# applied-ai-lab/genesis

Hardware: AMD Instinct MI355X
Metric: training images/sec (fwd+bwd+GECO step), GENESIS-V2 K=7 64x64 (higher is better)
Workload: dtype f32

## Files before the change

### genesis_amd/csrc/gx_kq.hip

```cpp
#include "gx_common.h"

#include <cstdlib>

#ifndef GX_KQ_ABL
#define GX_KQ_ABL 0
#endif
#ifndef GX_KQ_VAR
#define GX_KQ_VAR 0
#endif
#ifndef GX_QH_ABL
#define GX_QH_ABL 0
#endif

namespace {

enum { Q_C3 = 0, Q_DT0 = 1, Q_DT1 = 2, Q_DG = 3, Q_DT0H = 4, Q_DT1H = 5, Q_DGH = 6, Q_C3H = 7, Q_C5H = 8 };

template <int MODE> struct QCfg;
template <> struct QCfg<Q_C3> {
    static constexpr int NPH = 1, NT = 9, MAXT = 9, NCLS = 1;
    static constexpr bool PLANE_PER_PHASE = false;
    __host__ __device__ static constexpr int ntaps(int) { return 9; }
    __host__ __device__ static constexpr int tbase(int) { return 0; }
    __host__ __device__ static constexpr int ro(int, int i) { return i / 3; }
    __host__ __device__ static constexpr int co(int, int i) { return i % 3; }
    __host__ __device__ static constexpr int cls(int, int) { return 0; }
};
template <> struct QCfg<Q_DT0> {
    static constexpr int NPH = 3, NT = 15, MAXT = 5, NCLS = 2;
    static constexpr bool PLANE_PER_PHASE = false;
    __host__ __device__ static constexpr int ntaps(int) { return 5; }
    __host__ __device__ static constexpr int tbase(int p) { return 5 * p; }
    __host__ __device__ static constexpr int ro(int p, int) { return 2 - p; }
    __host__ __device__ static constexpr int co(int, int i) { return 2 - i / 2; }
    __host__ __device__ static constexpr int cls(int, int i) { return i & 1; }
};
template <> struct QCfg<Q_DT1> {
    static constexpr int NPH = 2, NT = 10, MAXT = 5, NCLS = 2;
    static constexpr bool PLANE_PER_PHASE = false;
    __host__ __device__ static constexpr int ntaps(int) { return 5; }
    __host__ __device__ static constexpr int tbase(int p) { return 5 * p; }
    __host__ __device__ static constexpr int ro(int p, int) { return 2 - p; }
    __host__ __device__ static constexpr int co(int, int i) { return 2 - i / 2; }
    __host__ __device__ static constexpr int cls(int, int i) { return i & 1; }
};
template <> struct QCfg<Q_DG> {
    static constexpr int NPH = 4, NT = 25, MAXT = 9, NCLS = 1;
    static constexpr bool PLANE_PER_PHASE = true;
    __host__ __device__ static constexpr int nkw(int p) { return 3 - (p & 1); }
    __host__ __device__ static constexpr int ntaps(int p) { return (3 - (p >> 1)) * (3 - (p & 1)); }
    __host__ __device__ static constexpr int tbase(int p) { return p == 0 ? 0 : (p == 1 ? 9 : (p == 2 ? 15 : 21)); }
    __host__ __device__ static constexpr int ro(int p, int i) { return i / nkw(p); }
    __host__ __device__ static constexpr int co(int p, int i) { return i % nkw(p); }
    __host__ __device__ static constexpr int cls(int, int) { return 0; }
};

template <int PA> struct QCfgDTH {
    static constexpr int NKH = PA ? 2 : 3;
    static constexpr int NPH = 2 * NKH, NT = 5 * NKH, MAXT = 3, NCLS = 2;
    static constexpr bool PLANE_PER_PHASE = false;
    __host__ __device__ static constexpr int ntaps(int ph) { return (ph & 1) ? 2 : 3; }
    __host__ __device__ static constexpr int tbase(int ph) { return 5 * (ph >> 1) + 3 * (ph & 1); }
    __host__ __device__ static constexpr int ro(int ph, int) { return 2 - (ph >> 1); }
    __host__ __device__ static constexpr int co(int ph, int j) { return 2 - (3 * (ph & 1) + j) / 2; }
// ... 136 lines not shown
    {                                                                                                  \
        const int toff_ = C::ro(PH, i_) * HS4 + C::co(PH, i_) * 4;                                     \
        _Pragma("unroll") for (int mi_ = 0; mi_ < MI; ++mi_)                                           \
            fa[set_][mi_] = *reinterpret_cast<const f32x4*>(wb + (i_) * 512 + a_lane + mi_ * 128);     \
        fb[set_][0] = *reinterpret_cast<const f32x4*>(ib + b_lane0 + toff_);                           \
        fb[set_][1] = *reinterpret_cast<const f32x4*>(ib + b_lane1 + toff_);                           \
    }
    GX_Q_READ(0, 0)
    __builtin_amdgcn_sched_group_barrier(0x100, 2 + MI, 0);
#pragma unroll
    for (int i = 0; i < nt; ++i) {
        const int cur = i & 1;
        if (i + 1 < nt) GX_Q_READ(i + 1, cur ^ 1)
        const int cl = C::cls(PH, i);
#pragma unroll
        for (int j = 0; j < 4; ++j) {
#pragma unroll
            for (int mi = 0; mi < MI; ++mi) {
                acc[cl][mi][0] = __builtin_amdgcn_mfma_f32_32x32x2f32(fa[cur][mi][j], fb[cur][0][j], acc[cl][mi][0], 0, 0, 0);
                acc[cl][mi][1] = __builtin_amdgcn_mfma_f32_32x32x2f32(fa[cur][mi][j], fb[cur][1][j], acc[cl][mi][1], 0, 0, 0);
            }
        }
#if GX_KQ_VAR == 1
        for (int r = 0; r < 4; ++r) {
            __builtin_amdgcn_sched_group_barrier(0x008, 4, 0);
            if (i + 1 < nt) __builtin_amdgcn_sched_group_barrier(0x100, 1, 0);
        }
#elif GX_KQ_VAR == 2
#else
        if (i + 1 < nt) __builtin_amdgcn_sched_group_barrier(0x100, 2 + MI, 0);
        __builtin_amdgcn_sched_group_barrier(0x008, 8 * MI, 0);
#endif
    }
#undef GX_Q_READ
}

__device__ __forceinline__ float q_amax_parts(const float* __restrict__ parts, int n) {
    float m = 0.f;
    int i0 = 0;
    if ((reinterpret_cast<uintptr_t>(parts) & 15) == 0) {
        const int n4 = n >> 2;
        for (int i = threadIdx.x & 63; i < n4; i += 64) {
            const f32x4 v = reinterpret_cast<const f32x4*>(parts)[i];
            m = fmaxf(fmaxf(m, fmaxf(v[0], v[1])), fmaxf(v[2], v[3]));
        }
        i0 = n4 << 2;
    }
    for (int i = i0 + (threadIdx.x & 63); i < n; i += 64) m = fmaxf(m, parts[i]);
#pragma unroll
    for (int o = 32; o > 0; o >>= 1) m = fmaxf(m, __shfl_xor(m, o, 64));
    return __builtin_bit_cast(float, __builtin_amdgcn_readfirstlane(__builtin_bit_cast(int, m)));
}

template <int MODE, int NQ, bool STATS, int MI = 2, int PF = PF_B6, bool TAP = false>
__device__ __forceinline__ void q_body(const float* __restrict__ in, const float* __restrict__ wp,
                                       const float* __restrict__ bias, float* __restrict__ out, const QGeom& g,
                                       float* lds, const int bx, const int by, const int par_a, const int mh = 0) {
    using C = QCfg<MODE>;
    constexpr bool F16 = PF == PF_F3, B1 = PF == PF_B1;
    constexpr bool B16 = MODE >= Q_DT0H;
    constexpr int NPH = C::NPH, NT = C::NT, MAXT = C::MAXT, NCLS = C::NCLS;
    constexpr int NW = (MAXT * 128 + 255) / 256;
    constexpr int WSLOT = NW * 1024;
    constexpr int ISLOT = NQ * 1024;

    const int tid = threadIdx.x, lane = tid & 63, wave = tid >> 6;
    const bool RT = MODE == Q_C3H && g.rt_tw > 0;
    const int TH = RT ? g.rt_th : 1 << g.lTH, TW = RT ? g.rt_tw : 1 << g.lTW, G = RT ? 1 : 1 << g.lG;
    constexpr int HL = MODE == Q_C5H ? 2 : 1;
    const int HS = TW + 2 * HL;
    const int CHS = G * (TH + 2 * HL) * HS;
    float* const ibuf0 = lds;
    float* const wbuf0 = lds + 2 * ISLOT;

    int tile = bx;
    const int tw_i = tile % g.tiles_w; tile /= g.tiles_w;
    const int th_i = tile % g.tiles_h; tile /= g.tiles_h;
    const int img0 = tile * G;
    const int R0 = th_i * TH, C0 = tw_i * TW;
    const int m0 = by * (MODE == Q_C3H ? 32 : 64);
    const int HiWi = g.Hi * g.Wi;

    const __amdgpu_buffer_rsrc_t in_rsrc = __builtin_amdgcn_make_buffer_rsrc(
        const_cast<float*>(in), 0, (int)((unsigned)g.N * (unsigned)g.K * (unsigned)HiWi * 4u), 0x00020000);
    const __amdgpu_buffer_rsrc_t w_rsrc = __builtin_amdgcn_make_buffer_rsrc(
        const_cast<float*>(wp), 0,
        B16 ? (int)((unsigned)NT * (unsigned)(g.K / 16) * gridDim.y * (unsigned)QHLay<MODE, PF>::TAPB)
            : (int)((unsigned)NT * (unsigned)g.K * gridDim.y * 256u), 0x00020000);
    int voff[NQ];
#pragma unroll
    for (int q = 0; q < NQ; ++q) {
        const int slot = tid + q * 256;
        const int quad = slot >= CHS ? 1 : 0;
        int rem = slot - quad * CHS;
        bool ok = slot < 2 * CHS;
        const int gi = rem / ((TH + 2 * HL) * HS); rem -= gi * (TH + 2 * HL) * HS;
        const int i = rem / HS;
        const int j = rem - i * HS;
        int row, col;
        if (MODE == Q_DG || MODE == Q_DGH) { row = 2 * (R0 + i) - 2; col = 2 * (C0 + j) - 2; }
        else { row = R0 - HL + i; col = C0 - HL + j; }
        ok = ok && img0 + gi < g.N && row >= 0 && row < g.Hi && col >= 0 && col < g.Wi;
        voff[q] = ok ? (((img0 + gi) * g.K + quad * (B16 ? 8 : 4)) * HiWi + row * g.Wi + col) * 4 : (int)0x80000000;
    }
    const int w_voff = tid * 16;
    const int w_sbase = by * g.nchunks * (NT * 2048);

    f32x16 acc[NCLS][MI][2];
#pragma unroll
    for (int c = 0; c < NCLS; ++c)
#pragma unroll
        for (int i = 0; i < MI; ++i)
#pragma unroll
            for (int j = 0; j < 2; ++j)
#pragma unroll
                for (int e = 0; e < 16; ++e) acc[c][i][j][e] = 0.f;
    int f16_sx = 0;
    if constexpr (B16 && F16) f16_sx = gx_f16_scale_exp(q_amax_parts(g.x_amax, g.x_amax_n));
    if constexpr (B16) {
        constexpr int TAPB = QHLay<MODE, PF>::TAPB;
        constexpr int NPL = QHLay<MODE, PF>::NP;
        constexpr int NWH = (MAXT * (TAPB / 16) + 255) / 256;
        constexpr int WSLOTB = NWH * 256 * 16;
        constexpr bool TRIM = NQ == 4 && MODE != Q_C3H;
        const int plane_bytes = TRIM ? 2 * CHS * 16 : NQ * 256 * 16;
        char* const ibuf = reinterpret_cast<char*>(lds);
        char* const wbufb = ibuf + NPL * plane_bytes;
        const int quad_l = lane >> 5;
        const int a_lane_b = (quad_l * QHLay<MODE, PF>::ROWS + (lane & 31)) * 16 + mh * 512;
        int b_lane_b[2];
#pragma unroll
        for (int nj = 0; nj < 2; ++nj) {
            const int p = wave * 64 + nj * 32 + (lane & 31);
            int c = p & (TW - 1);
            int r = (p >> g.lTW) & (TH - 1);
            int gi = p >> (g.lTW + g.lTH);
            if (RT) { gi = 0; r = p / TW; c = p - r * TW; if (r >= TH) { r = 0; c = 0; } }
            b_lane_b[nj] = (quad_l * CHS + (gi * (TH + 2 * HL) + r) * HS + c) * 16;
        }
        const int HS16 = HS * 16;
        const int nsc = g.K / 16;
        const int w_sbase = by * nsc * (NT * TAPB);
        float xin[NQ][8];
        f32x4 wreg[NWH];
#define GX_QH_LOAD_IN(sc_, plane_)                                                                     \
        {                                                                                              \
            const int po_ = MODE == Q_DGH ? (((plane_) >> 1) * g.Wi + ((plane_) & 1)) * 4 : 0;         \
            _Pragma("unroll") for (int q = 0; q < NQ; ++q)                                             \
                _Pragma("unroll") for (int e = 0; e < 8; ++e)                                          \
                    xin[q][e] = __builtin_bit_cast(float, __builtin_amdgcn_raw_buffer_load_b32(in_rsrc, voff[q], ((sc_) * 16 + e) * HiWi * 4 + po_, 0)); \
        }
#define GX_QH_STORE_IN()                                                                               \
        {                                                                                              \
            _Pragma("unroll") for (int q = 0; q < NQ; ++q) {                                           \
                q_bf16x8 ph_, pm_, pl_;                                                                \
                if (B1) {                                                                              \
                    _Pragma("unroll") for (int e = 0; e < 8; ++e) ph_[e] = (__bf16)xin[q][e];          \
                } else if (F16) {                                                                      \
                    q_f16x8 fh_, fl_;                                                                  \
                    _Pragma("unroll") for (int e = 0; e < 8; ++e) {                                    \
                        const float xs_ = ldexpf(xin[q][e], f16_sx);                                   \
                        const _Float16 h_ = (_Float16)xs_;                                             \
                        fh_[e] = h_; fl_[e] = (_Float16)(xs_ - (float)h_);                             \
                    }                                                                                  \
                    ph_ = __builtin_bit_cast(q_bf16x8, fh_); pm_ = __builtin_bit_cast(q_bf16x8, fl_);  \
                } else {                                                                               \
                _Pragma("unroll") for (int e = 0; e < 8; ++e) {                                        \
                    const __bf16 h_ = (__bf16)xin[q][e];                                               \
                    const float r1_ = xin[q][e] - (float)h_;                                           \
                    const __bf16 m_ = (__bf16)r1_;                                                     \
                    ph_[e] = h_; pm_[e] = m_; pl_[e] = (__bf16)(r1_ - (float)m_);                      \
                }                                                                                      \
                }                                                                                      \
                char* d_ = ibuf + (tid + q * 256) * 16;                                                \
                if (!TRIM || tid + q * 256 < 2 * CHS) {                                                \
                *reinterpret_cast<q_bf16x8*>(d_) = ph_;                                                \
                if (!B1) *reinterpret_cast<q_bf16x8*>(d_ + plane_bytes) = pm_;                         \
                if (!F16 && !B1) *reinterpret_cast<q_bf16x8*>(d_ + 2 * plane_bytes) = pl_;             \
                }                                                                                      \
            }                                                                                          \
        }
#define GX_QH_LOAD_W(sc_, ph_)                                                                         \
        {                                                                                              \
            const int so_ = w_sbase + ((sc_) * NT + C::tbase(ph_)) * TAPB;                             \
            _Pragma("unroll") for (int i = 0; i < NWH; ++i)                                            \
                wreg[i] = __builtin_bit_cast(f32x4, __builtin_amdgcn_raw_buffer_load_b128(w_rsrc, (tid + i * 256) * 16, so_, 0)); \
        }
#define GX_QH_STORE_W(dst_)                                                                            \
        {                                                                                              \
            _Pragma("unroll") for (int i = 0; i < NWH; ++i)                                            \
                *reinterpret_cast<f32x4*>((dst_) + (tid + i * 256) * 16) = wreg[i];                    \
        }
        GX_QH_LOAD_IN(0, 0)
        GX_QH_LOAD_W(0, 0)
        GX_QH_STORE_IN()
        GX_QH_STORE_W(wbufb)
#ifndef GX_QH_EARLY_DTH
#define GX_QH_EARLY_DTH 1
#endif
        constexpr bool EARLY_IN = MODE == Q_C3H || (GX_QH_EARLY_DTH && (MODE == Q_DT0H || MODE == Q_DT1H));
        constexpr bool ONE_W = MODE == Q_C3H;
        int s = 0;
        for (int sc = 0; sc < nsc; ++sc) {
            const bool last_chunk = sc + 1 == nsc;
#define GX_QH_STAGE(PH_)                                                                                         \
            {                                                                                                    \
                constexpr int NXT = (PH_) + 1 < NPH ? (PH_) + 1 : 0;                                             \
                constexpr bool last_ph = (PH_) + 1 == NPH;                                                       \
                const bool more = !last_ph || !last_chunk;                                                       \
                const bool in_next = C::newin(PH_) && more;         \
                __syncthreads();                                                                                 \
                if (more) GX_QH_LOAD_W(last_ph ? sc + 1 : sc, NXT)                                               \
                if (EARLY_IN) { if ((PH_) == 0 && !last_chunk && !(GX_QH_ABL & 8)) GX_QH_LOAD_IN(sc + 1, 0) }    \
                else if (in_next) GX_QH_LOAD_IN(last_ph ? sc + 1 : sc, C::plane(NXT))                            \
                q_phase_h<MODE, (PH_), NCLS, MI, PF>(acc, ibuf, wbufb + (ONE_W ? 0 : (s & 1)) * WSLOTB, plane_bytes, \
                                                 a_lane_b, b_lane_b[0], b_lane_b[1], HS16);                      \
                if (ONE_W) {                       \
                    if (more) { __syncthreads(); GX_QH_STORE_W(wbufb) }                                          \
                    if (in_next && !(GX_QH_ABL & 2)) GX_QH_STORE_IN()                                            \
                } else {                                                                                         \
                if (more) GX_QH_STORE_W(wbufb + ((s + 1) & 1) * WSLOTB)                                          \
                if (in_next) {                     \
                    __syncthreads();                                                                             \
                    if (!(GX_QH_ABL & 2)) GX_QH_STORE_IN()                                                       \
                }                                                                                                \
                }                                                                                                \
                ++s;                                                                                             \
            }
            GX_QH_STAGE(0)
            GX_QH_STAGE(1)
            GX_QH_STAGE(2)
            if constexpr (NPH > 3) GX_QH_STAGE(3)
            if constexpr (NPH > 4) { GX_QH_STAGE(4) GX_QH_STAGE(5) }
            if constexpr (NPH > 6) { GX_QH_STAGE(6) GX_QH_STAGE(7) GX_QH_STAGE(8) GX_QH_STAGE(9) }
#undef GX_QH_STAGE
        }
#undef GX_QH_LOAD_IN
#undef GX_QH_STORE_IN
#undef GX_QH_LOAD_W
#undef GX_QH_STORE_W
    } else {
    const int quad_l = lane >> 5;
    const int a_lane = (quad_l * 64 + (lane & 31)) * 4 + mh * 128;
    int b_lane[2];
#pragma unroll
    for (int nj = 0; nj < 2; ++nj) {
        const int p = wave * 64 + nj * 32 + (lane & 31);
        const int c = p & (TW - 1);
        const int r = (p >> g.lTW) & (TH - 1);
        const int gi = p >> (g.lTW + g.lTH);
        b_lane[nj] = (quad_l * CHS + (gi * (TH + 2 * HL) + r) * HS + c) * 4;
    }
    const int HS4 = HS * 4;


    f32x4 xin[NQ];
    f32x4 wreg[NW];
#if GX_KQ_ABL
    const long long abl_c0 = __builtin_readcyclecounter();
    const long long abl_w0 = wall_clock64();
#endif

#define GX_Q_LOAD_IN(chunk_, plane_)                                                                   \
    {                                                                                                  \
        const int so_ = ((chunk_) * 8 * HiWi + (MODE == Q_DG ? ((plane_) >> 1) * g.Wi + ((plane_) & 1) : 0)) * 4; \
        _Pragma("unroll") for (int q = 0; q < NQ; ++q) {                                               \
            _Pragma("unroll") for (int e = 0; e < 4; ++e)                                              \
                xin[q][e] = __builtin_bit_cast(float, __builtin_amdgcn_raw_buffer_load_b32(in_rsrc, voff[q], so_ + e * HiWi * 4, 0)); \
        }                                                                                              \
    }
#define GX_Q_STORE_IN(dst_)                                                                            \
    {                                                                                                  \
        _Pragma("unroll") for (int q = 0; q < NQ; ++q)                                                 \
            *reinterpret_cast<f32x4*>((dst_) + (tid + q * 256) * 4) = xin[q];                          \
    }
#define GX_Q_LOAD_W(chunk_, ph_)                                                                       \
    {                                                                                                  \
// ... 271 lines not shown
        __syncthreads();
#pragma unroll
        for (int i = 0; i < NB; ++i) { lds[i * 256 + tid] = st_s[i]; lds[(NB + i) * 256 + tid] = st_q[i]; }
        __syncthreads();
        const int vi = tid >> 4, sub = tid & 15;
        float v = 0.f;
        if (vi < 2 * NB) {
#pragma unroll
            for (int k = 0; k < 4; ++k) {
                const f32x4 r = *reinterpret_cast<const f32x4*>(lds + vi * 256 + sub * 16 + 4 * k);
                v += (r[0] + r[1]) + (r[2] + r[3]);
            }
        }
        v += __shfl_xor(v, 8, 64);
        v += __shfl_xor(v, 4, 64);
        v += __shfl_xor(v, 2, 64);
        v += __shfl_xor(v, 1, 64);
        if (sub == 0 && vi < 2 * NB) {
            const int part = (th_i * g.tiles_w + tw_i) * 2 + par_a;
            const int nblk = g.M >> 3;
            const int blk = (m0 >> 3) + mh * 4 + (vi % NB);
            if (blk < nblk && img0 < g.N)
                g.stats[(((size_t)img0 * g.stats_parts + part) * nblk + blk) * 2 + (vi / NB)] = v;
        }
    }
}

template <int MODE, int NQ>
__global__ void __launch_bounds__(256, 2)
kq_kernel(const float* __restrict__ in, const float* __restrict__ wp, const float* __restrict__ bias,
          float* __restrict__ out, QGeom g) {
    extern __shared__ __attribute__((aligned(16))) float lds[];
    const int bx = (int)blockIdx.x < g.nfull ? gx_xcd_tile(blockIdx.x, g.nfull) : (int)blockIdx.x;
    if (bx < g.nfull) q_body<MODE, NQ, false, 2>(in, wp, bias, out, g, lds, bx, blockIdx.y, 0);
    else q_body<MODE, NQ, false, 1>(in, wp, bias, out, g, lds, g.nfull + ((bx - g.nfull) >> 1), blockIdx.y, 0, (bx - g.nfull) & 1);
}

template <int NQ, bool STATS>
__global__ void __launch_bounds__(256, 2)
kq_dt_kernel(const float* __restrict__ in, const float* __restrict__ wp0, const float* __restrict__ wp1,
             const float* __restrict__ bias, float* __restrict__ out, QGeom g) {
    extern __shared__ __attribute__((aligned(16))) float lds[];
    const int bx = (int)blockIdx.x < g.nfull ? gx_xcd_tile(blockIdx.x, g.nfull) : (int)blockIdx.x;
    if (bx < g.nfull) {
        if (blockIdx.z) q_body<Q_DT1, NQ, STATS, 2>(in, wp1, bias, out, g, lds, bx, blockIdx.y, 1);
        else q_body<Q_DT0, NQ, STATS, 2>(in, wp0, bias, out, g, lds, bx, blockIdx.y, 0);
    } else {
        const int tile = g.nfull + ((bx - g.nfull) >> 1), mh = (bx - g.nfull) & 1;
        if (blockIdx.z) q_body<Q_DT1, NQ, STATS, 1>(in, wp1, bias, out, g, lds, tile, blockIdx.y, 1, mh);
        else q_body<Q_DT0, NQ, STATS, 1>(in, wp0, bias, out, g, lds, tile, blockIdx.y, 0, mh);
    }
}

template <int NQ, int PF = PF_B6>
__global__ void __launch_bounds__(256, 2)
kq_dgh_kernel(const float* __restrict__ in, const float* __restrict__ wp, float* __restrict__ out, QGeom g) {
    extern __shared__ __attribute__((aligned(16))) float lds[];
    const int bx = (int)blockIdx.x < g.nfull ? gx_xcd_tile(blockIdx.x, g.nfull) : (int)blockIdx.x;
    if (bx < g.nfull) q_body<Q_DGH, NQ, false, 2, PF>(in, wp, nullptr, out, g, lds, bx, blockIdx.y, 0);
    else q_body<Q_DGH, NQ, false, 1, PF>(in, wp, nullptr, out, g, lds, g.nfull + ((bx - g.nfull) >> 1), blockIdx.y, 0, (bx - g.nfull) & 1);
}

template <int NQ, int PF = PF_B6, bool TAP = false>
__global__ void __launch_bounds__(256, 3)
kq_c3h_kernel(const float* __restrict__ in, const float* __restrict__ wp, const float* __restrict__ bias,
              float* __restrict__ out, QGeom g) {
    extern __shared__ __attribute__((aligned(16))) float lds[];
    float* const tap4 = lds + g.tap_lds_off;
    if constexpr (TAP) {
        if ((threadIdx.x & 63) == 0) tap4[threadIdx.x >> 6] = 0.f;
    }
    for (int t = blockIdx.x; t < g.nfull; t += gridDim.x) {
        const int tile = gx_xcd_tile(t, g.nfull);
        q_body<Q_C3H, NQ, false, 1, PF, TAP>(in, wp, bias, out, g, lds, tile, blockIdx.y, 0, 0);
        __syncthreads();
    }
    if constexpr (TAP) {
        if (threadIdx.x == 0)
            g.o_amax[blockIdx.y * gridDim.x + blockIdx.x] = fmaxf(fmaxf(tap4[0], tap4[1]), fmaxf(tap4[2], tap4[3]));
    }
}

template <int NQ, int PF = PF_B6>
__global__ void __launch_bounds__(256, 2)
kq_c5h_kernel(const float* __restrict__ in, const float* __restrict__ wp, float* __restrict__ out, QGeom g) {
    extern __shared__ __attribute__((aligned(16))) float lds[];
    q_body<Q_C5H, NQ, false, 2, PF>(in, wp, nullptr, out, g, lds, gx_xcd_tile(blockIdx.x, gridDim.x), blockIdx.y, 0);
}

template <int NQ, bool STATS, int PF = PF_B6>
__global__ void __launch_bounds__(256, 2)
kq_dth_kernel(const float* __restrict__ in, const float* __restrict__ wp0, const float* __restrict__ wp1,
              const float* __restrict__ bias, float* __restrict__ out, QGeom g) {
    extern __shared__ __attribute__((aligned(16))) float lds[];
    int bxr = (int)blockIdx.x, z = (int)blockIdx.z;
    if (g.ilv) {
        const int gx = (int)gridDim.x >> 1, al = gx & ~7, b = (int)blockIdx.x;
        if (b < 2 * al) { z = (b >> 3) & 1; bxr = ((b >> 4) << 3) | (b & 7); }
        else { const int r = b - 2 * al, rem = gx - al; z = r / rem; bxr = al + r - z * rem; }
    }
    const int bx = bxr < g.nfull ? gx_xcd_tile(bxr, g.nfull) : bxr;
    if (bx < g.nfull) {
        if (z) q_body<Q_DT1H, NQ, STATS, 2, PF>(in, wp1, bias, out, g, lds, bx, blockIdx.y, 1);
        else q_body<Q_DT0H, NQ, STATS, 2, PF>(in, wp0, bias, out, g, lds, bx, blockIdx.y, 0);
    } else {
        const int tile = g.nfull + ((bx - g.nfull) >> 1), mh = (bx - g.nfull) & 1;
        if (z) q_body<Q_DT1H, NQ, STATS, 1, PF>(in, wp1, bias, out, g, lds, tile, blockIdx.y, 1, mh);
        else q_body<Q_DT0H, NQ, STATS, 1, PF>(in, wp0, bias, out, g, lds, tile, blockIdx.y, 0, mh);
    }
}

int q_ilog2(int v) { int l = 0; while ((1 << l) < v) ++l; return l; }

// ... 157 lines not shown
weight_amax_kernel(const float* __restrict__ w, int n, float* __restrict__ out) {
    const float r = gx_wg1024_amax(w, n);
    if (threadIdx.x == 0) out[0] = r;
}
int gx_kq_weight_amax_launch(const float* w, int n, float* out, hipStream_t s) {
    {
        GxProf pf(KID_SMALL_REDUCE, s, 0.0, 4.0 * n);
        hipLaunchKernelGGL(weight_amax_kernel, dim3(1), dim3(1024), 0, s, w, n, out);
    }
    GX_CHECK_LAUNCH("kq weight amax");
    return GX_OK;
}
static const int kFoldPartsAbove = 1024;
__global__ void __launch_bounds__(1024)
amax_fold2_kernel(const float* __restrict__ p0, int n0, const float* __restrict__ p1, int n1, float* __restrict__ out) {
    __shared__ float red[16];
    float m = 0.f;
    for (int i = threadIdx.x; i < n0; i += 1024) m = fmaxf(m, p0[i]);
    for (int i = threadIdx.x; i < n1; i += 1024) m = fmaxf(m, p1[i]);
#pragma unroll
    for (int o = 32; o > 0; o >>= 1) m = fmaxf(m, __shfl_xor(m, o, 64));
    if ((threadIdx.x & 63) == 0) red[threadIdx.x >> 6] = m;
    __syncthreads();
    if (threadIdx.x == 0) {
        float r = red[0];
#pragma unroll
        for (int i = 1; i < 16; ++i) r = fmaxf(r, red[i]);
        out[0] = r;
    }
}
static int kq_hint_parts(const float** parts, int* n, float* amax_ws, hipStream_t s) {
    const float *p0, *p1; int n0, n1;
    *parts = nullptr; *n = 0;
    if (!amax_ws || !gx_conv_input_hint(&p0, &n0, &p1, &n1)) return GX_OK;
    if (!p1 && n0 <= kFoldPartsAbove) { *parts = p0; *n = n0; return GX_OK; }
    {
        GxProf pf(KID_SMALL_REDUCE, s, 0.0, 4.0 * (n0 + n1));
        hipLaunchKernelGGL(amax_fold2_kernel, dim3(1), dim3(1024), 0, s, p0, n0, p1, p1 ? n1 : 0, amax_ws);
    }
    GX_CHECK_LAUNCH("kq amax fold (hint)");
    *parts = amax_ws; *n = 1;
    return GX_OK;
}
static int kq_fold_parts(const float** parts, int* n, float* amax_ws, hipStream_t s) {
    if (!*parts || *n <= kFoldPartsAbove || !amax_ws) return GX_OK;
    {
        GxProf pf(KID_SMALL_REDUCE, s, 0.0, 4.0 * *n);
        hipLaunchKernelGGL(weight_amax_kernel, dim3(1), dim3(1024), 0, s, *parts, *n, amax_ws);
    }
    GX_CHECK_LAUNCH("kq amax fold");
    *parts = amax_ws; *n = 1;
    return GX_OK;
}
static size_t qh_lds(const QGeom& g, int nq, int np = 3) {
    const int NWH = (3 * (np * 2048 / 16) + 255) / 256;
    const int CHS = (1 << g.lG) * ((1 << g.lTH) + 2) * ((1 << g.lTW) + 2);
    const size_t planes = nq == 4 ? (size_t)np * 2 * CHS * 16 : (size_t)np * nq * 256 * 16;
    const size_t lds = planes + (size_t)2 * NWH * 256 * 16;
    return lds <= 80 * 1024 ? lds : 0;
}
bool gx_kq_deconv_h_eligible(int N, int K, int M, int Hb, int Wb) {
    if (!kq_h_on() || K % 16 != 0 || !gx_kq_deconv_eligible(N, K, M, Hb, Wb, 2)) return false;
    QGeom g; int nq; size_t lds;
    return q_plan(N, K, M, Hb, Wb, Hb, Wb, 2 * Hb, 2 * Wb, &g, &nq, &lds, 5) && qh_lds(g, nq) > 0;
}
int gx_kq_deconv_fwd_h_launch(const float* in, const float* wp0, const float* wp1, const float* bias, float* out, int N,
                              int K, int M, int Hb, int Wb, float* stats, int* stats_parts, hipStream_t s, float* amax_ws,
                              const float* w_amax, const float* x_parts, int x_nparts) {
    QGeom g; int nq; size_t lds;
    if (!q_plan(N, K, M, Hb, Wb, Hb, Wb, 2 * Hb, 2 * Wb, &g, &nq, &lds, 5) || qh_lds(g, nq) == 0 || K % 16 != 0) {
        gx_set_error("kq deconv fwd (bf16 pipe): shape not eligible"); return GX_EINVAL;
    }
    const bool b1 = gx_kq_b1_on() && !amax_ws;
    lds = qh_lds(g, nq, b1 ? 1 : (amax_ws ? 2 : 3));
    const bool st = stats && g.lG == 0 && (M % 8) == 0;
    if (stats_parts) *stats_parts = 0;
    if (st) {
        g.stats = stats;
        g.stats_parts = g.tiles_h * g.tiles_w * 2;
        if (stats_parts) *stats_parts = g.stats_parts;
    }
    if (amax_ws && !x_parts) { const int rc = gx_kq_amax_launch(in, (size_t)N * K * Hb * Wb, amax_ws, s); if (rc) return rc; }
    else if (amax_ws) { const int rc = kq_fold_parts(&x_parts, &x_nparts, amax_ws, s); if (rc) return rc; }
    dim3 grid(1, gx_ceil_div(M, 64), 2);
    g.nfull = q_split_tail(g.tiles_h * g.tiles_w * gx_ceil_div(N, 1 << g.lG), M, &grid.x);
    if (grid.y == 1) { g.ilv = 1; grid.x *= 2; grid.z = 1; }
    {
        GxProf pf(KID_KQ_DTH, s, 2.0 * N * (double)M * K * 25 * Hb * Wb,
                  4.0 * ((double)N * K * Hb * Wb + (double)N * M * 4 * Hb * Wb + 25.0 * K * M));
        static bool a[12] = {false, false, false, false, false, false, false, false, false, false, false, false};
        q_note(GX_PLAN_KQ_DTH, amax_ws ? 2 : (b1 ? 3 : 1), g, nq, grid);
        if (amax_ws) {
            g.x_amax = x_parts ? x_parts : amax_ws;
            if (x_parts) g.x_amax_n = x_nparts;
            g.w_amax = w_amax;
            if (nq == 3 && st) { q_set_attr(&kq_dth_kernel<3, true, true>, &a[4]); hipLaunchKernelGGL((kq_dth_kernel<3, true, true>), grid, dim3(256), lds, s, in, wp0, wp1, bias, out, g); }
            else if (nq == 3) { q_set_attr(&kq_dth_kernel<3, false, true>, &a[5]); hipLaunchKernelGGL((kq_dth_kernel<3, false, true>), grid, dim3(256), lds, s, in, wp0, wp1, bias, out, g); }
            else if (st) { q_set_attr(&kq_dth_kernel<4, true, true>, &a[6]); hipLaunchKernelGGL((kq_dth_kernel<4, true, true>), grid, dim3(256), lds, s, in, wp0, wp1, bias, out, g); }
            else { q_set_attr(&kq_dth_kernel<4, false, true>, &a[7]); hipLaunchKernelGGL((kq_dth_kernel<4, false, true>), grid, dim3(256), lds, s, in, wp0, wp1, bias, out, g); }
        } else if (b1) {
            if (nq == 3 && st) { q_set_attr(&kq_dth_kernel<3, true, PF_B1>, &a[8]); hipLaunchKernelGGL((kq_dth_kernel<3, true, PF_B1>), grid, dim3(256), lds, s, in, wp0, wp1, bias, out, g); }
            else if (nq == 3) { q_set_attr(&kq_dth_kernel<3, false, PF_B1>, &a[9]); hipLaunchKernelGGL((kq_dth_kernel<3, false, PF_B1>), grid, dim3(256), lds, s, in, wp0, wp1, bias, out, g); }
            else if (st) { q_set_attr(&kq_dth_kernel<4, true, PF_B1>, &a[10]); hipLaunchKernelGGL((kq_dth_kernel<4, true, PF_B1>), grid, dim3(256), lds, s, in, wp0, wp1, bias, out, g); }
            else { q_set_attr(&kq_dth_kernel<4, false, PF_B1>, &a[11]); hipLaunchKernelGGL((kq_dth_kernel<4, false, PF_B1>), grid, dim3(256), lds, s, in, wp0, wp1, bias, out, g); }
        } else
        if (nq == 3 && st) { q_set_attr(&kq_dth_kernel<3, true>, &a[0]); hipLaunchKernelGGL((kq_dth_kernel<3, true>), grid, dim3(256), lds, s, in, wp0, wp1, bias, out, g); }
        else if (nq == 3) { q_set_attr(&kq_dth_kernel<3, false>, &a[1]); hipLaunchKernelGGL((kq_dth_kernel<3, false>), grid, dim3(256), lds, s, in, wp0, wp1, bias, out, g); }
        else if (st) { q_set_attr(&kq_dth_kernel<4, true>, &a[2]); hipLaunchKernelGGL((kq_dth_kernel<4, true>), grid, dim3(256), lds, s, in, wp0, wp1, bias, out, g); }
        else { q_set_attr(&kq_dth_kernel<4, false>, &a[3]); hipLaunchKernelGGL((kq_dth_kernel<4, false>), grid, dim3(256), lds, s, in, wp0, wp1, bias, out, g); }
    }
// ... 112 lines not shown
        else { const int rc = kq_fold_parts(&x_parts, &x_nparts, amax_ws, s); if (rc) return rc; }
    }
    dim3 grid(g.nfull, gx_ceil_div(M, 64));
    {
        GxProf pf(KID_KQ_C5H, s, 2.0 * N * (double)M * K * 25 * H * W, 4.0 * ((double)N * K * H * W + (double)N * M * H * W + 25.0 * K * M));
        static bool a4 = false, f4 = false, b4 = false;
        q_note(GX_PLAN_KQ_C5H, amax_ws ? 2 : (b1 ? 3 : 1), g, 4, grid);
        if (b1) {
            q_set_attr(&kq_c5h_kernel<4, PF_B1>, &b4);
            hipLaunchKernelGGL((kq_c5h_kernel<4, PF_B1>), grid, dim3(256), lds, s, in, wp, out, g);
        } else if (amax_ws) {
            g.x_amax = x_parts ? x_parts : amax_ws; g.w_amax = w_amax;
            if (x_parts) g.x_amax_n = x_nparts;
            q_set_attr(&kq_c5h_kernel<4, true>, &f4);
            hipLaunchKernelGGL((kq_c5h_kernel<4, true>), grid, dim3(256), lds, s, in, wp, out, g);
        } else {
        q_set_attr(&kq_c5h_kernel<4>, &a4);
        hipLaunchKernelGGL((kq_c5h_kernel<4>), grid, dim3(256), lds, s, in, wp, out, g);
        }
    }
    GX_CHECK_LAUNCH("kq conv5x5 (bf16 pipe)");
    return GX_OK;
}

bool gx_kq_deconv_dgrad_h_eligible(int N, int K, int M, int Hb, int Wb) {
    if (!kq_h_on() || K % 16 != 0 || !gx_kq_deconv_eligible(N, K, M, Hb, Wb, 1)) return false;
    QGeom g; int nq; size_t lds;
    return q_plan(N, K, M, Hb, Wb, 2 * Hb, 2 * Wb, Hb, Wb, &g, &nq, &lds, 9) && qh_lds(g, nq) > 0;
}
int gx_kq_deconv_dgrad_h_launch(const float* dy, const float* wp, float* dx, int N, int K, int M, int Hb, int Wb,
                                hipStream_t s, float* amax_ws, const float* w_amax, const float* x_parts, int x_nparts) {
    QGeom g; int nq; size_t lds;
    if (!q_plan(N, K, M, Hb, Wb, 2 * Hb, 2 * Wb, Hb, Wb, &g, &nq, &lds, 9) || qh_lds(g, nq) == 0 || K % 16 != 0) {
        gx_set_error("kq deconv dgrad (bf16 pipe): shape not eligible"); return GX_EINVAL;
    }
    const bool b1 = gx_kq_b1_on() && !amax_ws;
    lds = qh_lds(g, nq, b1 ? 1 : (amax_ws ? 2 : 3));
    if (amax_ws && !x_parts) { const int rc = gx_kq_amax_launch(dy, (size_t)N * K * 4 * Hb * Wb, amax_ws, s); if (rc) return rc; }
    else if (amax_ws) { const int rc = kq_fold_parts(&x_parts, &x_nparts, amax_ws, s); if (rc) return rc; }
    dim3 grid(1, gx_ceil_div(M, 64));
    g.nfull = q_split_tail(g.tiles_h * g.tiles_w * gx_ceil_div(N, 1 << g.lG), M, &grid.x);
    {
        GxProf pf(KID_KQ_DGH, s, 2.0 * N * (double)M * K * 25 * Hb * Wb,
                  4.0 * ((double)N * K * 4 * Hb * Wb + (double)N * M * Hb * Wb + 25.0 * K * M));
        static bool a3 = false, a4 = false, f3 = false, f4 = false, b3 = false, b4 = false;
        q_note(GX_PLAN_KQ_DGH, amax_ws ? 2 : (b1 ? 3 : 1), g, nq, grid);
        if (b1) {
            if (nq == 3) { q_set_attr(&kq_dgh_kernel<3, PF_B1>, &b3); hipLaunchKernelGGL((kq_dgh_kernel<3, PF_B1>), grid, dim3(256), lds, s, dy, wp, dx, g); }
            else { q_set_attr(&kq_dgh_kernel<4, PF_B1>, &b4); hipLaunchKernelGGL((kq_dgh_kernel<4, PF_B1>), grid, dim3(256), lds, s, dy, wp, dx, g); }
        } else if (amax_ws) {
            g.x_amax = x_parts ? x_parts : amax_ws;
            if (x_parts) g.x_amax_n = x_nparts;
            g.w_amax = w_amax;
            if (nq == 3) { q_set_attr(&kq_dgh_kernel<3, true>, &f3); hipLaunchKernelGGL((kq_dgh_kernel<3, true>), grid, dim3(256), lds, s, dy, wp, dx, g); }
            else { q_set_attr(&kq_dgh_kernel<4, true>, &f4); hipLaunchKernelGGL((kq_dgh_kernel<4, true>), grid, dim3(256), lds, s, dy, wp, dx, g); }
        } else
        if (nq == 3) { q_set_attr(&kq_dgh_kernel<3>, &a3); hipLaunchKernelGGL((kq_dgh_kernel<3>), grid, dim3(256), lds, s, dy, wp, dx, g); }
        else { q_set_attr(&kq_dgh_kernel<4>, &a4); hipLaunchKernelGGL((kq_dgh_kernel<4>), grid, dim3(256), lds, s, dy, wp, dx, g); }
    }
    GX_CHECK_LAUNCH("kq deconv dgrad (bf16 pipe)");
    return GX_OK;
}

int gx_kq_deconv_dgrad_launch(const float* dy, const float* wp, float* dx, int N, int K, int M, int Hb, int Wb,
                              hipStream_t s) {
    QGeom g; int nq; size_t lds;
    if (!q_plan(N, K, M, Hb, Wb, 2 * Hb, 2 * Wb, Hb, Wb, &g, &nq, &lds, 9)) { gx_set_error("kq deconv dgrad: shape not eligible"); return GX_EINVAL; }
    dim3 grid(1, gx_ceil_div(M, 64));
    g.nfull = q_split_tail(g.tiles_h * g.tiles_w * gx_ceil_div(N, 1 << g.lG), M, &grid.x);
    {
        GxProf pf(KID_TAPCONV_DG, s, 2.0 * N * (double)M * K * 25 * Hb * Wb,
                  4.0 * ((double)N * K * 4 * Hb * Wb + (double)N * M * Hb * Wb + 25.0 * K * M));
        static bool a3 = false, a4 = false;
        q_note(GX_PLAN_KQ_DG, 0, g, nq, grid);
        if (nq == 3) { q_set_attr(&kq_kernel<Q_DG, 3>, &a3); hipLaunchKernelGGL((kq_kernel<Q_DG, 3>), grid, dim3(256), lds, s, dy, wp, nullptr, dx, g); }
        else { q_set_attr(&kq_kernel<Q_DG, 4>, &a4); hipLaunchKernelGGL((kq_kernel<Q_DG, 4>), grid, dim3(256), lds, s, dy, wp, nullptr, dx, g); }
    }
    GX_CHECK_LAUNCH("kq deconv dgrad");
    return GX_OK;
}

extern "C" int gx_kq_precision(int mode) {
    GX_CHECK_ARG(mode >= -1 && mode <= 3, "gx_kq_precision: mode must be 0 (fp32 matrix pipe), 1 (bf16 pipe, six piece products), 2 (as 1, the transposed convs from three fp16 piece products), 3 (as 1, one bf16 piece per operand) or -1 (the environment's default)");
    g_kq_h = mode;
    return GX_OK;
}

extern "C" int gx_kq_policy(int mode) {
    GX_CHECK_ARG(mode >= 0 && mode <= 2, "gx_kq_policy: mode must be 0 (off), 1 (chip-filling layers) or 2 (every eligible shape)");
    g_kq_mode = mode;
    return GX_OK;
}
```

Before: 12160.

## Double-buffer input planes and prefetch weights two phases ahead in bf16 pipe

Adds a double-buffered input-plane variant of the fp16-split deconv data-gradient kernel, so the next plane is loaded and stored into the alternate LDS buffer while the current one is consumed, which removes one barrier per plane. It also adds a second weight register set so weights are prefetched two phases ahead for the DT0H/DT1H and DGH fp16 paths. The aim is to hide global-load latency behind MFMA work. The cost is twice the LDS for planes and more registers, which can reduce occupancy.

```diff
diff --git a/genesis_amd/csrc/gx_kq.hip b/genesis_amd/csrc/gx_kq.hip
--- a/genesis_amd/csrc/gx_kq.hip
+++ b/genesis_amd/csrc/gx_kq.hip
@@ -10,6 +10,15 @@
 #endif
 #ifndef GX_QH_ABL
 #define GX_QH_ABL 0
+#endif
+#ifndef GX_QH_DGH_DB
+#define GX_QH_DGH_DB 2
+#endif
+#ifndef GX_QH_W2
+#define GX_QH_W2 1
+#endif
+#ifndef GX_QH_W2_DGH3
+#define GX_QH_W2_DGH3 0
 #endif
 
 namespace {
@@ -252,7 +261,8 @@
     return __builtin_bit_cast(float, __builtin_amdgcn_readfirstlane(__builtin_bit_cast(int, m)));
 }
 
-template <int MODE, int NQ, bool STATS, int MI = 2, int PF = PF_B6, bool TAP = false>
+template <int MODE> constexpr int qh_prow(int ph) { if constexpr (MODE == Q_DGH) return QCfg<Q_DGH>::prow(ph); else return 0; }
+template <int MODE, int NQ, bool STATS, int MI = 2, int PF = PF_B6, bool TAP = false, bool DB = false>
 __device__ __forceinline__ void q_body(const float* __restrict__ in, const float* __restrict__ wp,
                                        const float* __restrict__ bias, float* __restrict__ out, const QGeom& g,
                                        float* lds, const int bx, const int by, const int par_a, const int mh = 0) {
@@ -324,8 +334,13 @@
         constexpr int WSLOTB = NWH * 256 * 16;
         constexpr bool TRIM = NQ == 4 && MODE != Q_C3H;
         const int plane_bytes = TRIM ? 2 * CHS * 16 : NQ * 256 * 16;
+        constexpr bool DBI = DB && MODE == Q_DGH && F16;
+        static_assert(!DB || DBI, "double-buffered planes: the fp16 x 3 data gradient only");
+        constexpr bool W2 = GX_QH_W2 && F16 && NPH % 2 == 0 &&
+                            (((MODE == Q_DT0H || MODE == Q_DT1H) && NQ == 3) || (MODE == Q_DGH && (DBI || (GX_QH_W2_DGH3 && NQ == 3))));
         char* const ibuf = reinterpret_cast<char*>(lds);
-        char* const wbufb = ibuf + NPL * plane_bytes;
+        const int ibuf_bytes = NPL * plane_bytes;
+        char* const wbufb = ibuf + (DBI ? 2 : 1) * ibuf_bytes;
         const int quad_l = lane >> 5;
         const int a_lane_b = (quad_l * QHLay<MODE, PF>::ROWS + (lane & 31)) * 16 + mh * 512;
         int b_lane_b[2];
@@ -342,7 +357,7 @@
         const int nsc = g.K / 16;
         const int w_sbase = by * nsc * (NT * TAPB);
         float xin[NQ][8];
-        f32x4 wreg[NWH];
+        f32x4 wreg[W2 ? 2 : 1][NWH];
 #define GX_QH_LOAD_IN(sc_, plane_)                                                                     \
         {                                                                                              \
             const int po_ = MODE == Q_DGH ? (((plane_) >> 1) * g.Wi + ((plane_) & 1)) * 4 : 0;         \
@@ -350,7 +365,7 @@
                 _Pragma("unroll") for (int e = 0; e < 8; ++e)                                          \
                     xin[q][e] = __builtin_bit_cast(float, __builtin_amdgcn_raw_buffer_load_b32(in_rsrc, voff[q], ((sc_) * 16 + e) * HiWi * 4 + po_, 0)); \
         }
-#define GX_QH_STORE_IN()                                                                               \
+#define GX_QH_STORE_IN(dst_)                                                                           \
         {                                                                                              \
             _Pragma("unroll") for (int q = 0; q < NQ; ++q) {                                           \
                 q_bf16x8 ph_, pm_, pl_;                                                                \
@@ -372,7 +387,7 @@
                     ph_[e] = h_; pm_[e] = m_; pl_[e] = (__bf16)(r1_ - (float)m_);                      \
                 }                                                                                      \
                 }                                                                                      \
-                char* d_ = ibuf + (tid + q * 256) * 16;                                                \
+                char* d_ = (dst_) + (tid + q * 256) * 16;                                              \
                 if (!TRIM || tid + q * 256 < 2 * CHS) {                                                \
                 *reinterpret_cast<q_bf16x8*>(d_) = ph_;                                                \
                 if (!B1) *reinterpret_cast<q_bf16x8*>(d_ + plane_bytes) = pm_;                         \
@@ -380,25 +395,30 @@
                 }                                                                                      \
             }                                                                                          \
         }
-#define GX_QH_LOAD_W(sc_, ph_)                                                                         \
+#define GX_QH_LOAD_W(set_, sc_, ph_)                                                                   \
         {                                                                                              \
             const int so_ = w_sbase + ((sc_) * NT + C::tbase(ph_)) * TAPB;                             \
             _Pragma("unroll") for (int i = 0; i < NWH; ++i)                                            \
-                wreg[i] = __builtin_bit_cast(f32x4, __builtin_amdgcn_raw_buffer_load_b128(w_rsrc, (tid + i * 256) * 16, so_, 0)); \
-        }
-#define GX_QH_STORE_W(dst_)                                                                            \
+                wreg[set_][i] = __builtin_bit_cast(f32x4, __builtin_amdgcn_raw_buffer_load_b128(w_rsrc, (tid + i * 256) * 16, so_, 0)); \
+        }
+#define GX_QH_STORE_W(set_, dst_)                                                                      \
         {                                                                                              \
             _Pragma("unroll") for (int i = 0; i < NWH; ++i)                                            \
-                *reinterpret_cast<f32x4*>((dst_) + (tid + i * 256) * 16) = wreg[i];                    \
+                *reinterpret_cast<f32x4*>((dst_) + (tid + i * 256) * 16) = wreg[set_][i];              \
         }
         GX_QH_LOAD_IN(0, 0)
-        GX_QH_LOAD_W(0, 0)
-        GX_QH_STORE_IN()
-        GX_QH_STORE_W(wbufb)
+        GX_QH_LOAD_W(0, 0, 0)
+        GX_QH_STORE_IN(ibuf)
+        GX_QH_STORE_W(0, wbufb)
+        if constexpr (W2) GX_QH_LOAD_W(1, 0, 1)
 #ifndef GX_QH_EARLY_DTH
 #define GX_QH_EARLY_DTH 1
 #endif
-        constexpr bool EARLY_IN = MODE == Q_C3H || (GX_QH_EARLY_DTH && (MODE == Q_DT0H || MODE == Q_DT1H));
+#ifndef GX_QH_EARLY_C5H
+#define GX_QH_EARLY_C5H 0
+#endif
+        constexpr bool EARLY_IN = MODE == Q_C3H || (GX_QH_EARLY_DTH && (MODE == Q_DT0H || MODE == Q_DT1H)) ||
+                                  (GX_QH_EARLY_C5H && MODE == Q_C5H);
         constexpr bool ONE_W = MODE == Q_C3H;
         int s = 0;
         for (int sc = 0; sc < nsc; ++sc) {
@@ -409,20 +429,32 @@
                 constexpr bool last_ph = (PH_) + 1 == NPH;                                                       \
                 const bool more = !last_ph || !last_chunk;                                                       \
                 const bool in_next = C::newin(PH_) && more;         \
+                 \
+                constexpr int N2 = ((PH_) + 2) % NPH;                                                            \
+                constexpr bool wrap2 = (PH_) + 2 >= NPH;                                                         \
+                constexpr int LSET = W2 ? ((PH_) & 1) : 0, SSET = W2 ? (((PH_) + 1) & 1) : 0;                     \
+                                                                               \
+                constexpr int PL = C::plane(PH_), PROW = qh_prow<MODE>(PH_);                                     \
+                const bool pl_next = DBI && (PL < 3 || !last_chunk);                                             \
                 __syncthreads();                                                                                 \
-                if (more) GX_QH_LOAD_W(last_ph ? sc + 1 : sc, NXT)                                               \
-                if (EARLY_IN) { if ((PH_) == 0 && !last_chunk && !(GX_QH_ABL & 8)) GX_QH_LOAD_IN(sc + 1, 0) }    \
+                if constexpr (W2) { if (!wrap2 || !last_chunk) GX_QH_LOAD_W(LSET, wrap2 ? sc + 1 : sc, N2) }     \
+                else if (more) GX_QH_LOAD_W(0, last_ph ? sc + 1 : sc, NXT)                                       \
+                if (DBI) { if (PROW == 0 && pl_next && !(GX_QH_ABL & 8)) GX_QH_LOAD_IN(PL == 3 ? sc + 1 : sc, (PL + 1) & 3) } \
+                else if (EARLY_IN) { if ((PH_) == 0 && !last_chunk && !(GX_QH_ABL & 8)) GX_QH_LOAD_IN(sc + 1, 0) } \
                 else if (in_next) GX_QH_LOAD_IN(last_ph ? sc + 1 : sc, C::plane(NXT))                            \
-                q_phase_h<MODE, (PH_), NCLS, MI, PF>(acc, ibuf, wbufb + (ONE_W ? 0 : (s & 1)) * WSLOTB, plane_bytes, \
+                q_phase_h<MODE, (PH_), NCLS, MI, PF>(acc, ibuf + (DBI ? (PL & 1) * ibuf_bytes : 0),              \
+                                                 wbufb + (ONE_W ? 0 : (s & 1)) * WSLOTB, plane_bytes,            \
                                                  a_lane_b, b_lane_b[0], b_lane_b[1], HS16);                      \
                 if (ONE_W) {                       \
-                    if (more) { __syncthreads(); GX_QH_STORE_W(wbufb) }                                          \
-                    if (in_next && !(GX_QH_ABL & 2)) GX_QH_STORE_IN()                                            \
+                    if (more) { __syncthreads(); GX_QH_STORE_W(0, wbufb) }                                       \
+                    if (in_next && !(GX_QH_ABL & 2)) GX_QH_STORE_IN(ibuf)                                        \
                 } else {                                                                                         \
-                if (more) GX_QH_STORE_W(wbufb + ((s + 1) & 1) * WSLOTB)                                          \
-                if (in_next) {                     \
+                if (more) GX_QH_STORE_W(SSET, wbufb + ((s + 1) & 1) * WSLOTB)                                    \
+                if (DBI) {                                                                                       \
+                    if (PROW == 1 && pl_next && !(GX_QH_ABL & 2)) GX_QH_STORE_IN(ibuf + ((PL + 1) & 1) * ibuf_bytes) \
+                } else if (in_next) {              \
                     __syncthreads();                                                                             \
-                    if (!(GX_QH_ABL & 2)) GX_QH_STORE_IN()                                                       \
+                    if (!(GX_QH_ABL & 2)) GX_QH_STORE_IN(ibuf)                                                   \
                 }                                                                                                \
                 }                                                                                                \
                 ++s;                                                                                             \
@@ -800,13 +832,13 @@
     }
 }
 
-template <int NQ, int PF = PF_B6>
+template <int NQ, int PF = PF_B6, bool DB = false>
 __global__ void __launch_bounds__(256, 2)
 kq_dgh_kernel(const float* __restrict__ in, const float* __restrict__ wp, float* __restrict__ out, QGeom g) {
     extern __shared__ __attribute__((aligned(16))) float lds[];
     const int bx = (int)blockIdx.x < g.nfull ? gx_xcd_tile(blockIdx.x, g.nfull) : (int)blockIdx.x;
-    if (bx < g.nfull) q_body<Q_DGH, NQ, false, 2, PF>(in, wp, nullptr, out, g, lds, bx, blockIdx.y, 0);
-    else q_body<Q_DGH, NQ, false, 1, PF>(in, wp, nullptr, out, g, lds, g.nfull + ((bx - g.nfull) >> 1), blockIdx.y, 0, (bx - g.nfull) & 1);
+    if (bx < g.nfull) q_body<Q_DGH, NQ, false, 2, PF, false, DB>(in, wp, nullptr, out, g, lds, bx, blockIdx.y, 0);
+    else q_body<Q_DGH, NQ, false, 1, PF, false, DB>(in, wp, nullptr, out, g, lds, g.nfull + ((bx - g.nfull) >> 1), blockIdx.y, 0, (bx - g.nfull) & 1);
 }
 
 template <int NQ, int PF = PF_B6, bool TAP = false>
@@ -1070,10 +1102,10 @@
     *parts = amax_ws; *n = 1;
     return GX_OK;
 }
-static size_t qh_lds(const QGeom& g, int nq, int np = 3) {
+static size_t qh_lds(const QGeom& g, int nq, int np = 3, int nbuf = 1) {
     const int NWH = (3 * (np * 2048 / 16) + 255) / 256;
     const int CHS = (1 << g.lG) * ((1 << g.lTH) + 2) * ((1 << g.lTW) + 2);
-    const size_t planes = nq == 4 ? (size_t)np * 2 * CHS * 16 : (size_t)np * nq * 256 * 16;
+    const size_t planes = (size_t)nbuf * (nq == 4 ? (size_t)np * 2 * CHS * 16 : (size_t)np * nq * 256 * 16);
     const size_t lds = planes + (size_t)2 * NWH * 256 * 16;
     return lds <= 80 * 1024 ? lds : 0;
 }
@@ -1292,6 +1324,13 @@
             g.x_amax = x_parts ? x_parts : amax_ws;
             if (x_parts) g.x_amax_n = x_nparts;
             g.w_amax = w_amax;
+#if GX_QH_DGH_DB
+            static bool d3 = false, d4 = false;
+            const size_t lds_db = GX_QH_DGH_DB >= 2 || (size_t)grid.x * grid.y <= 2 * 256 ? qh_lds(g, nq, 2, 2) : 0;
+            if (lds_db > 0 && nq == 3) { q_set_attr(&kq_dgh_kernel<3, PF_F3, true>, &d3); hipLaunchKernelGGL((kq_dgh_kernel<3, PF_F3, true>), grid, dim3(256), lds_db, s, dy, wp, dx, g); }
+            else if (lds_db > 0) { q_set_attr(&kq_dgh_kernel<4, PF_F3, true>, &d4); hipLaunchKernelGGL((kq_dgh_kernel<4, PF_F3, true>), grid, dim3(256), lds_db, s, dy, wp, dx, g); }
+            else
+#endif
             if (nq == 3) { q_set_attr(&kq_dgh_kernel<3, true>, &f3); hipLaunchKernelGGL((kq_dgh_kernel<3, true>), grid, dim3(256), lds, s, dy, wp, dx, g); }
             else { q_set_attr(&kq_dgh_kernel<4, true>, &f4); hipLaunchKernelGGL((kq_dgh_kernel<4, true>), grid, dim3(256), lds, s, dy, wp, dx, g); }
         } else
```

New measurement: 12380, median of 6. 1.02x the previous value.
